# LessUp/n-body

Measured on AMD Instinct MI355X. Metric: pair_interactions_per_s, higher is better.
Workload: dtype f32; 1 GPU; plummer_N1048576_direct_n2_velocity_verlet; bodies=1048576, seed=42, deterministic=True, deterministic_mode=1

## Files before the change

n-body_amd/csrc/api.hip:

```cpp

#include <cstdarg>
#include <cstdlib>
#include <cstring>

#include "common.h"
#include "onesweep.h"

namespace nbh {

static thread_local char g_err[512] = "";

void set_error(const char* fmt, ...) {
  va_list ap;
  va_start(ap, fmt);
  vsnprintf(g_err, sizeof(g_err), fmt, ap);
  va_end(ap);
}

int fail(nbody_hip_status code, const char* file, int line, const char* fmt, ...) {
  char msg[384];
  va_list ap;
  va_start(ap, fmt);
  vsnprintf(msg, sizeof(msg), fmt, ap);
  va_end(ap);
  const char* base = strrchr(file, '/');
  snprintf(g_err, sizeof(g_err), "%s at %s:%d", msg, base ? base + 1 : file, line);
  return (int)code;
}

int Workspace::reserve(size_t want) {
  if (want <= bytes) return NBODY_HIP_OK;
  size_t cap = bytes + bytes / 2;
  if (cap < want) cap = want;
  cap = (cap + 255) & ~(size_t)255;
  want = (want + 255) & ~(size_t)255;
  if (ptr) {
    NBH_HIP(hipDeviceSynchronize());
    NBH_HIP(hipFree(ptr));
    ptr = nullptr;
    bytes = 0;
    generation++;
  }
  void* p = nullptr;
  hipError_t e = hipMalloc(&p, cap);
  if (e != hipSuccess && cap > want) {
    (void)hipGetLastError();
    cap = want;
    e = hipMalloc(&p, cap);
  }
  if (e != hipSuccess) {
    (void)hipGetLastError();
    return ::nbh::fail(e == hipErrorOutOfMemory ? NBODY_HIP_ERR_RESOURCE : NBODY_HIP_ERR_DEVICE, __FILE__, __LINE__,
                       "hipMalloc(%zu bytes of workspace): %s", cap, hipGetErrorString(e));
  }
  ptr = p;
  bytes = cap;
  generation++;
  return NBODY_HIP_OK;
}

void Workspace::release() {
  if (ptr) (void)hipFree(ptr);
  ptr = nullptr;
  bytes = 0;
  generation++;
}

}

using namespace nbh;

extern "C" int nbody_hip_abi_version(void) { return NBODY_HIP_ABI_VERSION; }

extern "C" int nbody_hip_sort_info(int* driver_compiled, int* self_test, int* own_self_test, int* rocprim_version) {
  if (driver_compiled) *driver_compiled = NBH_ONESWEEP_AVAILABLE;
  if (self_test) *self_test = nbh::driver_sort_verdict.state.load(std::memory_order_acquire);
  if (own_self_test) *own_self_test = nbh::own_sort_verdict.state.load(std::memory_order_acquire);
  if (rocprim_version) *rocprim_version = (int)ROCPRIM_VERSION;
  return NBODY_HIP_OK;
}

extern "C" const char* nbody_hip_last_error(void) { return g_err; }

extern "C" int nbody_hip_device_count(void) {
  int n = 0;
  if (hipGetDeviceCount(&n) != hipSuccess) {
    (void)hipGetLastError();
    return 0;
  }
  return n;
}

extern "C" int nbody_hip_ctx_create(nbody_hip_ctx** out, int device, void* stream) {
  if (!out) return NBH_FAIL(NBODY_HIP_ERR_STATE, "null output pointer");
  *out = nullptr;
  const int ndev = nbody_hip_device_count();
  if (ndev <= 0)
    return NBH_FAIL(NBODY_HIP_ERR_DEVICE, "no HIP device available (this library has no CPU fallback)");
  if (device < 0 || device >= ndev)
    return NBH_FAIL(NBODY_HIP_ERR_VALIDATION, "device %d out of range [0,%d)", device, ndev);
  NBH_HIP(hipSetDevice(device));
  nbody_hip_ctx* c = new nbody_hip_ctx();
  c->device = device;
  c->stream = static_cast<hipStream_t>(stream);
  hipError_t e = hipHostMalloc(reinterpret_cast<void**>(&c->host_scalar), 4 * sizeof(double), hipHostMallocDefault);
  if (e == hipSuccess) e = hipEventCreate(&c->ev0);
  if (e == hipSuccess) e = hipEventCreate(&c->ev1);
  if (e != hipSuccess) {
    nbody_hip_ctx_destroy(c);
    return NBH_FAIL(NBODY_HIP_ERR_DEVICE, "context resources: %s", hipGetErrorString(e));
  }
  *out = c;
  return NBODY_HIP_OK;
}

extern "C" int nbody_hip_ctx_destroy(nbody_hip_ctx* ctx) {
  if (!ctx) return NBODY_HIP_OK;
  NBH_DESTROY_BEGIN
  (void)hipSetDevice(ctx->device);
  (void)hipStreamSynchronize(ctx->stream);
  ctx->posm.release();
  ctx->partial.release();
  ctx->reduce.release();
  if (ctx->host_scalar) (void)hipHostFree(ctx->host_scalar);
  if (ctx->ev0) (void)hipEventDestroy(ctx->ev0);
  if (ctx->ev1) (void)hipEventDestroy(ctx->ev1);
  if (ctx->capture_stream) (void)hipStreamDestroy(ctx->capture_stream);
  delete ctx;
  NBH_DESTROY_END
}

extern "C" int nbody_hip_ctx_set_stream(nbody_hip_ctx* ctx, void* stream) {
  if (!ctx) return NBH_FAIL(NBODY_HIP_ERR_STATE, "null context");
  ctx->stream = static_cast<hipStream_t>(stream);
  return NBODY_HIP_OK;
}

extern "C" int nbody_hip_ctx_synchronize(nbody_hip_ctx* ctx) {
  if (!ctx) return NBH_FAIL(NBODY_HIP_ERR_STATE, "null context");
  NBH_NOT_CAPTURABLE(ctx, "nbody_hip_ctx_synchronize");
  NBH_HIP(hipSetDevice(ctx->device));
  NBH_HIP(hipStreamSynchronize(ctx->stream));
  return NBODY_HIP_OK;
}


struct nbody_hip_graph {
  nbody_hip_ctx* ctx = nullptr;
  hipGraph_t graph = nullptr;
  hipGraphExec_t exec = nullptr;
  unsigned long long generation = 0;
};

extern "C" int nbody_hip_capture_begin(nbody_hip_ctx* ctx) {
  if (!ctx) return NBH_FAIL(NBODY_HIP_ERR_STATE, "null context");
  if (ctx->capturing) return NBH_FAIL(NBODY_HIP_ERR_STATE, "capture already in progress");
  NBH_HIP(hipSetDevice(ctx->device));
  if (!ctx->capture_stream) NBH_HIP(hipStreamCreateWithFlags(&ctx->capture_stream, hipStreamNonBlocking));
  NBH_HIP(hipStreamSynchronize(ctx->stream));
  NBH_HIP(hipStreamBeginCapture(ctx->capture_stream, hipStreamCaptureModeThreadLocal));
  ctx->user_stream = ctx->stream;
  ctx->stream = ctx->capture_stream;
  ctx->capturing = true;
  ctx->capture_failed = false;
  return NBODY_HIP_OK;
}

extern "C" int nbody_hip_capture_end(nbody_hip_ctx* ctx, nbody_hip_graph** out) {
  if (!ctx || !out) return NBH_FAIL(NBODY_HIP_ERR_STATE, "null argument");
  *out = nullptr;
  if (!ctx->capturing) return NBH_FAIL(NBODY_HIP_ERR_STATE, "no capture in progress");
  hipGraph_t graph = nullptr;
  const hipError_t e = hipStreamEndCapture(ctx->capture_stream, &graph);
  ctx->stream = ctx->user_stream;
  ctx->capturing = false;
  if (e != hipSuccess || !graph || ctx->capture_failed) {
    (void)hipGetLastError();
    if (graph) (void)hipGraphDestroy(graph);
    return NBH_FAIL(NBODY_HIP_ERR_DEVICE, "hipStreamEndCapture: %s (a call inside the capture was not capturable)",
                    hipGetErrorString(e));
  }
  nbody_hip_graph* g = new nbody_hip_graph();
  g->ctx = ctx;
  g->graph = graph;
  g->generation = ctx->generation();
  const hipError_t ei = hipGraphInstantiate(&g->exec, graph, nullptr, nullptr, 0);
  if (ei != hipSuccess) {
    (void)hipGraphDestroy(graph);
    delete g;
    return NBH_FAIL(NBODY_HIP_ERR_DEVICE, "hipGraphInstantiate: %s", hipGetErrorString(ei));
  }
  *out = g;
  return NBODY_HIP_OK;
}

extern "C" int nbody_hip_graph_launch(nbody_hip_graph* g, int times) {
  if (!g || !g->exec) return NBH_FAIL(NBODY_HIP_ERR_STATE, "null graph");
  if (g->ctx->capturing) return NBH_FAIL(NBODY_HIP_ERR_STATE, "graph launch inside a capture");
  if (g->generation != g->ctx->generation())
    return NBH_FAIL(NBODY_HIP_ERR_STATE, "step graph is stale: device buffers of its context were re-allocated "
                    "after it was recorded (record it again)");
  NBH_HIP(hipSetDevice(g->ctx->device));
  g->ctx->graph_replays += (unsigned long long)(times > 0 ? times : 0);
  for (int i = 0; i < times; i++) NBH_HIP(hipGraphLaunch(g->exec, g->ctx->stream));
  return NBODY_HIP_OK;
}

extern "C" int nbody_hip_graph_destroy(nbody_hip_graph* g) {
  if (!g) return NBODY_HIP_OK;
  NBH_DESTROY_BEGIN
  (void)hipSetDevice(g->ctx->device);
  (void)hipStreamSynchronize(g->ctx->stream);
  if (g->exec) (void)hipGraphExecDestroy(g->exec);
  if (g->graph) (void)hipGraphDestroy(g->graph);
  delete g;
  NBH_DESTROY_END
}


static inline float** field(nbody_particle_data* d, int k) { return &d->pos_x + k; }
static inline float* const* cfield(const nbody_particle_data* d, int k) { return &d->pos_x + k; }

extern "C" int nbody_hip_particles_alloc(nbody_particle_data* d, size_t count) {
  if (!d) return NBH_FAIL(NBODY_HIP_ERR_STATE, "null particle data");
  if (count == 0) return NBH_FAIL(NBODY_HIP_ERR_VALIDATION, "Particle count must be greater than 0");
  if (count > 100000000u)
    return NBH_FAIL(NBODY_HIP_ERR_VALIDATION, "Particle count exceeds maximum supported (100M)");
  if (nbody_hip_device_count() <= 0)
    return NBH_FAIL(NBODY_HIP_ERR_DEVICE, "no HIP device available (this library has no CPU fallback)");
  const size_t stride = ((count * sizeof(float)) + 255) & ~(size_t)255;
  char* base = nullptr;
  NBH_HIP(hipMalloc(reinterpret_cast<void**>(&base), stride * 13));
  hipError_t e = hipMemset(base, 0, stride * 13);
  if (e != hipSuccess) {
    (void)hipFree(base);
    return NBH_FAIL(NBODY_HIP_ERR_DEVICE, "hipMemset: %s", hipGetErrorString(e));
  }
  for (int k = 0; k < 13; k++) *field(d, k) = reinterpret_cast<float*>(base + stride * k);
  d->count = count;
  return NBODY_HIP_OK;
}

extern "C" int nbody_hip_particles_free(nbody_particle_data* d) {
  if (!d) return NBODY_HIP_OK;
  if (d->pos_x) {
    NBH_HIP(hipDeviceSynchronize());
    NBH_HIP(hipFree(d->pos_x));
  }
  for (int k = 0; k < 13; k++) *field(d, k) = nullptr;
  d->count = 0;
  return NBODY_HIP_OK;
}

static const int kCopied[10] = {0, 1, 2, 3, 4, 5, 6, 7, 8, 12};

extern "C" int nbody_hip_particles_upload(nbody_particle_data* d, const nbody_particle_data* h) {
  if (!d || !h) return NBH_FAIL(NBODY_HIP_ERR_STATE, "null particle data");
  if (h->count > d->count)
    return NBH_FAIL(NBODY_HIP_ERR_VALIDATION, "host count %zu exceeds device capacity %zu", h->count, d->count);
  const size_t bytes = h->count * sizeof(float);
  for (int k : kCopied) {
    if (!*cfield(h, k) || !*cfield(d, k)) return NBH_FAIL(NBODY_HIP_ERR_STATE, "null array in particle data");
    NBH_HIP(hipMemcpy(*field(d, k), *cfield(h, k), bytes, hipMemcpyHostToDevice));
  }
  return NBODY_HIP_OK;
}

extern "C" int nbody_hip_particles_download(nbody_particle_data* h, const nbody_particle_data* d) {
  if (!d || !h) return NBH_FAIL(NBODY_HIP_ERR_STATE, "null particle data");
  if (d->count > h->count)
    return NBH_FAIL(NBODY_HIP_ERR_VALIDATION, "device count %zu exceeds host capacity %zu", d->count, h->count);
  const size_t bytes = d->count * sizeof(float);
  for (int k : kCopied) {
    if (!*cfield(h, k) || !*cfield(d, k)) return NBH_FAIL(NBODY_HIP_ERR_STATE, "null array in particle data");
    NBH_HIP(hipMemcpy(*field(h, k), *cfield(d, k), bytes, hipMemcpyDeviceToHost));
  }
  return NBODY_HIP_OK;
}


extern "C" int nbody_hip_pack_posm(nbody_hip_ctx* ctx, const float* x, const float* y,
                                   const float* z, const float* mass, size_t count,
                                   nbody_float4* out) {
  if (!ctx) return NBH_FAIL(NBODY_HIP_ERR_STATE, "null context");
  if (count == 0) return NBODY_HIP_OK;
  if (!x || !y || !z || !mass || !out) return NBH_FAIL(NBODY_HIP_ERR_STATE, "null argument");
  if (count > 0x3fffffffu) return NBH_FAIL(NBODY_HIP_ERR_VALIDATION, "body count exceeds 2^30");
  NBH_HIP(hipSetDevice(ctx->device));
  return pack_posm(ctx, x, y, z, mass, count, reinterpret_cast<float4*>(out));
}

namespace nbh {
__global__ __launch_bounds__(kBlock) void unpack3_kernel(const float4* __restrict__ in, int n,
                                                         float* __restrict__ x,
                                                         float* __restrict__ y,
                                                         float* __restrict__ z) {
  const int i = blockIdx.x * kBlock + threadIdx.x;
  if (i < n) {
    const float4 v = in[i];
    x[i] = v.x; y[i] = v.y; z[i] = v.z;
  }
}
}

extern "C" int nbody_hip_unpack3(nbody_hip_ctx* ctx, const nbody_float4* in, size_t count, float* x,
                                 float* y, float* z) {
  if (!ctx) return NBH_FAIL(NBODY_HIP_ERR_STATE, "null context");
  if (count == 0) return NBODY_HIP_OK;
  if (!x || !y || !z || !in) return NBH_FAIL(NBODY_HIP_ERR_STATE, "null argument");
  if (count > 0x3fffffffu) return NBH_FAIL(NBODY_HIP_ERR_VALIDATION, "body count exceeds 2^30");
  NBH_HIP(hipSetDevice(ctx->device));
  hipLaunchKernelGGL(unpack3_kernel, dim3((unsigned)((count + kBlock - 1) / kBlock)), dim3(kBlock),
                     0, ctx->stream, reinterpret_cast<const float4*>(in), (int)count, x, y, z);
  NBH_LAUNCH_CHECK();
  return NBODY_HIP_OK;
}

extern "C" int nbody_hip_direct_forces(nbody_hip_ctx* ctx, const nbody_particle_data* d, float G,
                                       float eps2, int block_size) {
  if (!ctx) return NBH_FAIL(NBODY_HIP_ERR_STATE, "null context");
  if (!d) return NBH_FAIL(NBODY_HIP_ERR_STATE, "null particle data");
  if (block_size <= 0 || block_size > 1024)
    return NBH_FAIL(NBODY_HIP_ERR_VALIDATION, "CUDA block size must be between 1 and 1024");
  const size_t n = d->count;
  if (n == 0) return NBODY_HIP_OK;
  if (!d->pos_x || !d->pos_y || !d->pos_z || !d->mass || !d->acc_x || !d->acc_y || !d->acc_z)
    return NBH_FAIL(NBODY_HIP_ERR_STATE, "particle data has null arrays");
  if (n > 0x3fffffffu) return NBH_FAIL(NBODY_HIP_ERR_VALIDATION, "body count exceeds 2^30");
  NBH_HIP(hipSetDevice(ctx->device));
  if (int rc = ctx->posm.reserve(n * sizeof(float4))) return rc;
  float4* posm = static_cast<float4*>(ctx->posm.ptr);
  if (int rc = pack_posm(ctx, d->pos_x, d->pos_y, d->pos_z, d->mass, n, posm)) return rc;
  return direct_packed(ctx, posm, n, posm, n, G, eps2, nullptr, 0, d->acc_x, d->acc_y, d->acc_z,
                       nullptr, nullptr, nullptr, nullptr, nullptr, nullptr, 0.f);
}

extern "C" int nbody_hip_direct_forces_packed(nbody_hip_ctx* ctx, const nbody_float4* targets,
                                              size_t n_targets, const nbody_float4* sources,
                                              size_t n_sources, nbody_float4* acc_out, float G,
                                              float eps2, int accumulate) {
  if (!ctx) return NBH_FAIL(NBODY_HIP_ERR_STATE, "null context");
  if (n_targets == 0) return NBODY_HIP_OK;
  if (!targets || !acc_out || (n_sources > 0 && !sources))
    return NBH_FAIL(NBODY_HIP_ERR_STATE, "null argument");
  NBH_HIP(hipSetDevice(ctx->device));
  return direct_packed(ctx, reinterpret_cast<const float4*>(targets), n_targets,
                       reinterpret_cast<const float4*>(sources), n_sources, G, eps2,
                       reinterpret_cast<float4*>(acc_out), accumulate, nullptr, nullptr, nullptr,
                       nullptr, nullptr, nullptr, nullptr, nullptr, nullptr, 0.f);
}

extern "C" int nbody_hip_direct_forces_pair_packed(nbody_hip_ctx* ctx, const nbody_float4* a, size_t n_a,
                                                   const nbody_float4* b, size_t n_b, nbody_float4* acc_a,
                                                   int accumulate_a, nbody_float4* acc_b, int accumulate_b,
                                                   float G, float eps2) {
  if (!ctx) return NBH_FAIL(NBODY_HIP_ERR_STATE, "null context");
  if (n_a == 0 || n_b == 0) return NBH_FAIL(NBODY_HIP_ERR_VALIDATION, "both body sets must be non-empty");
  if (!a || !b || !acc_a || !acc_b) return NBH_FAIL(NBODY_HIP_ERR_STATE, "null argument");
  if (n_a > 0x3fffffffu || n_b > 0x3fffffffu) return NBH_FAIL(NBODY_HIP_ERR_VALIDATION, "body count exceeds 2^30");
  if (!(eps2 >= 1e-12f))
    return NBH_FAIL(NBODY_HIP_ERR_VALIDATION, "pair evaluation needs eps2 >= 1e-12 (use the one-sided entry point)");
  NBH_HIP(hipSetDevice(ctx->device));
  return direct_symmetric_pair(ctx, reinterpret_cast<const float4*>(a), n_a, reinterpret_cast<const float4*>(b),
                               n_b, G, eps2, reinterpret_cast<float4*>(acc_a), accumulate_a,
                               reinterpret_cast<float4*>(acc_b), accumulate_b);
}

extern "C" int nbody_hip_time_direct_packed(nbody_hip_ctx* ctx, const nbody_float4* targets,
                                            size_t n_targets, const nbody_float4* sources,
                                            size_t n_sources, nbody_float4* acc_out, float G,
                                            float eps2, int iters, float* ms_per_launch) {
  if (!ctx) return NBH_FAIL(NBODY_HIP_ERR_STATE, "null context");
  if (!ms_per_launch || iters <= 0) return NBH_FAIL(NBODY_HIP_ERR_VALIDATION, "bad timing arguments");
  NBH_HIP(hipSetDevice(ctx->device));
  if (int rc = nbody_hip_direct_forces_packed(ctx, targets, n_targets, sources, n_sources, acc_out, G, eps2, 0))
    return rc;
  NBH_HIP(hipEventRecord(ctx->ev0, ctx->stream));
  for (int i = 0; i < iters; i++)
    if (int rc = nbody_hip_direct_forces_packed(ctx, targets, n_targets, sources, n_sources, acc_out, G, eps2, 0))
      return rc;
  NBH_HIP(hipEventRecord(ctx->ev1, ctx->stream));
  NBH_HIP(hipEventSynchronize(ctx->ev1));
  float ms = 0.f;
  NBH_HIP(hipEventElapsedTime(&ms, ctx->ev0, ctx->ev1));
  *ms_per_launch = ms / (float)iters;
  return NBODY_HIP_OK;
}

extern "C" int nbody_hip_direct_deterministic(nbody_hip_ctx* ctx, int mode) {
  if (!ctx) return NBH_FAIL(NBODY_HIP_ERR_STATE, "null context");
  if (mode < 0 || mode > 2) return NBH_FAIL(NBODY_HIP_ERR_VALIDATION, "mode must be 0 (atomics), 1 (slots when they fit) or 2 (slots required)");
  ctx->deterministic = mode;
  if (mode == 0 && ctx->partial.bytes > ((size_t)64 << 20) && !ctx->capturing) {
    NBH_HIP(hipSetDevice(ctx->device));
    NBH_HIP(hipDeviceSynchronize());
    ctx->partial.release();
  }
  return NBODY_HIP_OK;
}

extern "C" int nbody_hip_direct_slot_budget(nbody_hip_ctx* ctx, unsigned long long bytes) {
  if (!ctx) return NBH_FAIL(NBODY_HIP_ERR_STATE, "null context");
  ctx->det_budget = bytes ? (size_t)bytes : ((size_t)24 << 30);
  return NBODY_HIP_OK;
}

extern "C" int nbody_hip_direct_info(nbody_hip_ctx* ctx, size_t count, float eps2, nbody_hip_direct_info_t* out) {
  if (!out) return NBH_FAIL(NBODY_HIP_ERR_STATE, "null argument");
  const nbody_hip_ctx defaults{};
  const nbody_hip_ctx* c = ctx ? ctx : &defaults;
  memset(out, 0, sizeof(*out));
  out->deterministic_mode = c->deterministic;
  out->last_kernel = c->last_direct_kernel;
  out->workspace_bytes_held = c->partial.bytes;
  if (count == 0) return NBODY_HIP_OK;
  if (count > 0x3fffffffu) return NBH_FAIL(NBODY_HIP_ERR_VALIDATION, "body count exceeds 2^30");
  const bool dev = ctx && nbody_hip_device_count() > 0 && hipSetDevice(ctx->device) == hipSuccess;
  DirectPlan p = direct_plan(c, count, dev);
  if (!(eps2 >= 1e-12f)) p.symmetric = false;
  if (!p.symmetric) {
    out->kernel = 0;
    return NBODY_HIP_OK;
  }
  out->kernel = p.det ? 2 : 1;
  out->bodies_per_lane_equal = p.eq.R;
  out->bodies_per_lane_general = p.gen.R;
  out->reaction_slots = p.det ? p.eq.D : 0;
  out->iside_slots = p.det ? p.eq.splits : 1;
  out->workspace_bytes_needed = p.bytes;
  out->slot_bytes_wanted = p.det_bytes_wanted;
  return NBODY_HIP_OK;
}

extern "C" int nbody_hip_direct_tuning(nbody_hip_ctx* ctx, int variant, int targets_per_lane,
                                       int source_splits) {
  if (!ctx) return NBH_FAIL(NBODY_HIP_ERR_STATE, "null context");
  if (variant < -1 || variant > 3) return NBH_FAIL(NBODY_HIP_ERR_VALIDATION, "variant must be -1 (auto), 0, 1, 2 or 3");
  if (targets_per_lane != 0 && targets_per_lane != 1 && targets_per_lane != 2 && targets_per_lane != 4 &&
      targets_per_lane != 6 && targets_per_lane != 8 && targets_per_lane != 12 && targets_per_lane != 16)
    return NBH_FAIL(NBODY_HIP_ERR_VALIDATION, "targets_per_lane must be 0 (auto), 1, 2, 4 (6, 8, 16: symmetric kernel only)");
  if (source_splits < 0 || source_splits > 4096)
    return NBH_FAIL(NBODY_HIP_ERR_VALIDATION, "source_splits must be in [0, 4096]");
  ctx->tune_variant = variant;
  ctx->tune_tpl = targets_per_lane;
  ctx->tune_splits = source_splits;
  return NBODY_HIP_OK;
}
```

n-body_amd/csrc/direct_sym.hip:

```cpp

#include <type_traits>

#include "common.h"

namespace nbh {

typedef float f2 __attribute__((ext_vector_type(2)));

__device__ __forceinline__ float wave_rot1(float v) {
  return __int_as_float(__builtin_amdgcn_mov_dpp(__float_as_int(v), 0x134 , 0xF, 0xF, false));
}

constexpr int kSymBlocksPerCU = 16;
constexpr int kSymMinChunks = 4;
constexpr float kFar = 1.0e18f;

template <int R, bool RECT, bool EQM, bool DET = false>
__global__ __launch_bounds__(kBlock) void direct_sym_kernel(const float4* __restrict__ posm, int n,
                                                            const float4* __restrict__ posj, int nj,
                                                            int NB, int NBJ, int chunks_per_split,
                                                            double* __restrict__ acc64,
                                                            void* __restrict__ accj,
                                                            size_t plane_i, size_t plane_j,
                                                            const unsigned int* __restrict__ mass_range,
                                                            float eps2) {
  const bool uniform = mass_range[0] == mass_range[1] && mass_range[2] == mass_range[3] &&
                       mass_range[0] == mass_range[2] && ordered_to_float(mass_range[0]) > 0.f;
  if (uniform != EQM) return;
  const float m0 = EQM ? ordered_to_float(mass_range[0]) : 1.0f;
  constexpr int S = kBlock * R;
  __shared__ float slab[2][4][3][64];
  const int tid = threadIdx.x, lane = tid & 63, w = tid >> 6;
  const int A = blockIdx.x;
  const int D = RECT ? NBJ - 1 : NB / 2;
  constexpr int CPB = kBlock * R / 64;
  const int q0 = blockIdx.y * chunks_per_split;
  const int q1 = min((D + 1) * CPB, q0 + chunks_per_split);
  if (q0 >= q1) {
    if constexpr (DET) {
#pragma unroll
      for (int r = 0; r < R; r++)
#pragma unroll
        for (int c = 0; c < 3; c++)
          acc64[((size_t)blockIdx.y * 3 + c) * plane_i + (size_t)(A * S + r * kBlock + tid)] = 0.0;
    }
    return;
  }

  f2 xi[R / 2], yi[R / 2], zi[R / 2], mi[R / 2];
#pragma unroll
  for (int r = 0; r < R / 2; r++) {
    float4 p0 = make_float4(kFar, kFar, kFar, 0.f), p1 = p0;
    const int i0 = A * S + (2 * r) * kBlock + tid, i1 = i0 + kBlock;
    if (i0 < n) p0 = posm[i0];
    if (i1 < n) p1 = posm[i1];
    xi[r] = f2{p0.x, p1.x}; yi[r] = f2{p0.y, p1.y}; zi[r] = f2{p0.z, p1.z}; mi[r] = f2{p0.w, p1.w};
  }
  constexpr bool LACC = R >= 8;
  constexpr int RR = LACC ? 1 : R;
  __shared__ double lacc[LACC ? 3 * R * kBlock : 1];
  double sx[RR], sy[RR], sz[RR];
  if constexpr (LACC) {
#pragma unroll
    for (int k = 0; k < 3 * R; k++) lacc[k * kBlock + tid] = 0.0;
  } else {
#pragma unroll
    for (int r = 0; r < R; r++) sx[r] = sy[r] = sz[r] = 0.0;
  }
  f2 ax[R / 2], ay[R / 2], az[R / 2];
#pragma unroll
  for (int r = 0; r < R / 2; r++) ax[r] = ay[r] = az[r] = f2{0.f, 0.f};
  const f2 e2 = {eps2, eps2};

  auto partner_valid = [&](int d) { return RECT || !((NB % 2 == 0) && d == D && d > 0 && A >= D); };
  const int nchunks = q1 - q0;

  auto load_chunk = [&](int q) -> float4 {
    const int d = (q0 + q) / CPB, c = (q0 + q) % CPB;
    const int B = RECT ? d : (A + d) % NB;
    const int j = B * S + c * 64 + lane;
    float4 p = make_float4(kFar, kFar, kFar, 0.f);
    if (RECT) { if (j < nj) p = posj[j]; }
    else if (j < n && partner_valid(d)) p = posm[j];
    return p;
  };
  auto flush_chunk = [&](int q) {
    const int pd = (q0 + q) / CPB, pc = (q0 + q) % CPB;
    if constexpr (DET) {
      if (RECT || pd > 0) {
        const size_t plane = RECT ? plane_j : plane_i;
        float* slot = static_cast<float*>(accj) + (size_t)(RECT ? A : pd - 1) * 3 * plane;
        const unsigned int j = (unsigned int)((RECT ? pd : (A + pd) % NB) * S + pc * 64 + lane), pl = (unsigned int)plane;
        const int sb = q & 1;
        const bool keep = partner_valid(pd);
#pragma unroll
        for (int c = 0; c < 3; c++) {
          const float v = (slab[sb][0][c][lane] + slab[sb][1][c][lane]) + (slab[sb][2][c][lane] + slab[sb][3][c][lane]);
          slot[c * pl + j] = keep ? v : 0.f;
        }
      }
    } else if ((RECT || pd > 0) && partner_valid(pd)) {
      const int j = (RECT ? pd : (A + pd) % NB) * S + pc * 64 + lane;
      const int sb = q & 1;
      double* dst = RECT ? static_cast<double*>(accj) : acc64;
      const size_t plane = RECT ? plane_j : plane_i;
#pragma unroll
      for (int c = 0; c < 3; c++) {
        const float v = (slab[sb][0][c][lane] + slab[sb][1][c][lane]) + (slab[sb][2][c][lane] + slab[sb][3][c][lane]);
        unsafeAtomicAdd(&dst[c * plane + (size_t)j], (double)v * (double)m0);
      }
    }
  };

  float4 jnext = load_chunk(0);
  for (int q = 0; q < nchunks; q++) {
    const float4 jcur = jnext;
    if (q + 1 < nchunks) jnext = load_chunk(q + 1);
    const int d = (q0 + q) / CPB;
    const bool react = RECT || d > 0;
    if (q > 0) {
      __syncthreads();
      if (w == (q & 3)) flush_chunk(q - 1);
    }
    float jx = jcur.x, jy = jcur.y, jz = jcur.z, jm = jcur.w;
    float hjx = 0.f, hjy = 0.f, hjz = 0.f;
    auto steps = [&](auto react_tag) {
      constexpr bool REACT = decltype(react_tag)::value;
      constexpr int kStepUnroll = R >= 16 ? 1 : 2;
#pragma unroll kStepUnroll
      for (int k = 0; k < 64; k++) {
        const f2 sxj = {jx, jx}, syj = {jy, jy}, szj = {jz, jz}, smj = {jm, jm};
        f2 dx[R / 2], dy[R / 2], dz[R / 2], g[R / 2];
#pragma unroll
        for (int r = 0; r < R / 2; r++) {
          dx[r] = sxj - xi[r]; dy[r] = syj - yi[r]; dz[r] = szj - zi[r];
          g[r] = __builtin_elementwise_fma(dx[r], dx[r], __builtin_elementwise_fma(dy[r], dy[r], __builtin_elementwise_fma(dz[r], dz[r], e2)));
        }
#pragma unroll
        for (int r = 0; r < R / 2; r++) {
          g[r].x = __builtin_amdgcn_rsqf(g[r].x);
          g[r].y = __builtin_amdgcn_rsqf(g[r].y);
        }
#pragma unroll
        for (int r = 0; r < R / 2; r++) g[r] = (g[r] * g[r]) * g[r];
        f2 hx = {hjx, 0.f}, hy = {hjy, 0.f}, hz = {hjz, 0.f};
#pragma unroll
        for (int r = 0; r < R / 2; r++) {
          const f2 fj = EQM ? g[r] : g[r] * smj;
          ax[r] = __builtin_elementwise_fma(fj, dx[r], ax[r]);
          ay[r] = __builtin_elementwise_fma(fj, dy[r], ay[r]);
          az[r] = __builtin_elementwise_fma(fj, dz[r], az[r]);
          if (REACT) {
            const f2 fi = EQM ? g[r] : g[r] * mi[r];
            hx = __builtin_elementwise_fma(-fi, dx[r], hx);
            hy = __builtin_elementwise_fma(-fi, dy[r], hy);
            hz = __builtin_elementwise_fma(-fi, dz[r], hz);
          }
        }
        if (REACT) {
          hjx = wave_rot1(hx.x + hx.y); hjy = wave_rot1(hy.x + hy.y); hjz = wave_rot1(hz.x + hz.y);
        }
        jx = wave_rot1(jx); jy = wave_rot1(jy); jz = wave_rot1(jz); jm = wave_rot1(jm);
      }
    };
    if constexpr (R >= 12 && !EQM) {
      (void)react;
      steps(std::true_type{});
    } else {
      if (react) steps(std::true_type{}); else steps(std::false_type{});
    }
    slab[q & 1][w][0][lane] = hjx; slab[q & 1][w][1][lane] = hjy; slab[q & 1][w][2][lane] = hjz;
    if ((q & 3) == 3 || q == nchunks - 1) {
#pragma unroll
      for (int r = 0; r < R / 2; r++) {
        if constexpr (LACC) {
          lacc[(0 * R + 2 * r) * kBlock + tid] += (double)ax[r].x; lacc[(0 * R + 2 * r + 1) * kBlock + tid] += (double)ax[r].y;
          lacc[(1 * R + 2 * r) * kBlock + tid] += (double)ay[r].x; lacc[(1 * R + 2 * r + 1) * kBlock + tid] += (double)ay[r].y;
          lacc[(2 * R + 2 * r) * kBlock + tid] += (double)az[r].x; lacc[(2 * R + 2 * r + 1) * kBlock + tid] += (double)az[r].y;
        } else {
          sx[2 * r] += (double)ax[r].x; sx[2 * r + 1] += (double)ax[r].y;
          sy[2 * r] += (double)ay[r].x; sy[2 * r + 1] += (double)ay[r].y;
          sz[2 * r] += (double)az[r].x; sz[2 * r + 1] += (double)az[r].y;
        }
        ax[r] = ay[r] = az[r] = f2{0.f, 0.f};
      }
    }
  }
  __syncthreads();
  if (w == (nchunks & 3)) flush_chunk(nchunks - 1);
#pragma unroll
  for (int r = 0; r < R; r++) {
    const int i = A * S + r * kBlock + tid;
    const double fx = LACC ? lacc[(0 * R + r) * kBlock + tid] : sx[LACC ? 0 : r];
    const double fy = LACC ? lacc[(1 * R + r) * kBlock + tid] : sy[LACC ? 0 : r];
    const double fz = LACC ? lacc[(2 * R + r) * kBlock + tid] : sz[LACC ? 0 : r];
    if constexpr (DET) {
      double* slot = acc64 + (size_t)blockIdx.y * 3 * plane_i;
      const unsigned int iu = (unsigned int)i, pl = (unsigned int)plane_i;
      slot[iu] = fx;
      slot[pl + iu] = fy;
      slot[2u * pl + iu] = fz;
    } else {
      unsafeAtomicAdd(&acc64[(size_t)i], fx * (double)m0);
      unsafeAtomicAdd(&acc64[plane_i + (size_t)i], fy * (double)m0);
      unsafeAtomicAdd(&acc64[2 * plane_i + (size_t)i], fz * (double)m0);
    }
  }
}

__global__ void mass_range_init_kernel(unsigned int* enc) {
  if (threadIdx.x < 4) enc[threadIdx.x] = (threadIdx.x & 1) ? 0u : 0xffffffffu;
}

__global__ __launch_bounds__(kBlock) void mass_range_kernel(const float4* __restrict__ posm, int n,
                                                            unsigned int* __restrict__ enc) {
  __shared__ float red[4][2];
  float lo = INFINITY, hi = -INFINITY;
  for (int i = blockIdx.x * kBlock + threadIdx.x; i < n; i += gridDim.x * kBlock) {
    const float m = posm[i].w;
    lo = fminf(lo, m); hi = fmaxf(hi, m);
  }
#pragma unroll
  for (int off = 32; off > 0; off >>= 1) {
    lo = fminf(lo, __shfl_down(lo, off, 64));
    hi = fmaxf(hi, __shfl_down(hi, off, 64));
  }
  const int w = threadIdx.x >> 6;
  if ((threadIdx.x & 63) == 0) { red[w][0] = lo; red[w][1] = hi; }
  __syncthreads();
  if (threadIdx.x == 0) {
    for (int k = 1; k < 4; k++) { lo = fminf(lo, red[k][0]); hi = fmaxf(hi, red[k][1]); }
    atomicMin(&enc[0], float_to_ordered(fminf(lo, red[0][0])));
    atomicMax(&enc[1], float_to_ordered(fmaxf(hi, red[0][1])));
  }
}

struct SlotLayout {
  const double* isl;
  const float* rsl;
  size_t plane;
  int n_i, n_r;
};

__global__ __launch_bounds__(kBlock) void direct_sym_finalize_kernel(
    SlotLayout eq, SlotLayout gen, int apply_m0, const unsigned int* __restrict__ mass_range, int n, float G,
    float4* __restrict__ acc4, int accumulate, float* __restrict__ ax, float* __restrict__ ay, float* __restrict__ az,
    float* __restrict__ vx, float* __restrict__ vy, float* __restrict__ vz, const float* __restrict__ aox,
    const float* __restrict__ aoy, const float* __restrict__ aoz, float half_dt) {
  const int i = blockIdx.x * kBlock + threadIdx.x;
  if (i >= n) return;
  SlotLayout L = eq;
  double m0 = 1.0;
  if (mass_range) {
    const bool uniform = mass_range[0] == mass_range[1] && mass_range[2] == mass_range[3] &&
                         mass_range[0] == mass_range[2] && ordered_to_float(mass_range[0]) > 0.f;
    if (!uniform) L = gen;
    else if (apply_m0) m0 = (double)ordered_to_float(mass_range[0]);
  }
  double sx = 0.0, sy = 0.0, sz = 0.0;
  for (int k = 0; k < L.n_r; k++) {
    const float* p = L.rsl + (size_t)k * 3 * L.plane;
    sx += (double)p[i]; sy += (double)p[L.plane + i]; sz += (double)p[2 * L.plane + i];
  }
  for (int k = 0; k < L.n_i; k++) {
    const double* p = L.isl + (size_t)k * 3 * L.plane;
    sx += p[i]; sy += p[L.plane + i]; sz += p[2 * L.plane + i];
  }
  const double gm = (double)G * m0;
  const float fx = (float)(gm * sx), fy = (float)(gm * sy), fz = (float)(gm * sz);
  if (acc4) {
    float4 o = make_float4(fx, fy, fz, 0.f);
    if (accumulate) { const float4 c = acc4[i]; o.x += c.x; o.y += c.y; o.z += c.z; }
    acc4[i] = o;
  } else {
    ax[i] = fx; ay[i] = fy; az[i] = fz;
    if (vx) {
      vx[i] = kick1(vx[i], aox[i], fx, half_dt);
      vy[i] = kick1(vy[i], aoy[i], fy, half_dt);
      vz[i] = kick1(vz[i], aoz[i], fz, half_dt);
    }
  }
}

static void launch_mass_range(nbody_hip_ctx* ctx, const float4* pi, int ni, const float4* pj, int nj,
                              unsigned int* enc) {
  hipLaunchKernelGGL(mass_range_init_kernel, dim3(1), dim3(64), 0, ctx->stream, enc);
  const int bi = (ni + kBlock - 1) / kBlock, bj = (nj + kBlock - 1) / kBlock;
  hipLaunchKernelGGL(mass_range_kernel, dim3(bi < 256 ? bi : 256), dim3(kBlock), 0, ctx->stream, pi, ni, enc);
  hipLaunchKernelGGL(mass_range_kernel, dim3(bj < 256 ? bj : 256), dim3(kBlock), 0, ctx->stream, pj, nj, enc + 2);
}

template <int R, bool RECT, bool DET>
static void launch_sym(nbody_hip_ctx* ctx, dim3 grid, const float4* pi, int ni, const float4* pj, int nj,
                       int NB, int NBJ, int per, double* acci, void* accj, const unsigned int* enc,
                       float eps2) {
  const size_t S = (size_t)kBlock * R;
  hipLaunchKernelGGL((direct_sym_kernel<R, RECT, true, DET>), grid, dim3(kBlock), 0, ctx->stream, pi, ni, pj, nj,
                     NB, NBJ, per, acci, accj, (size_t)NB * S, (size_t)NBJ * S, enc, eps2);
  hipLaunchKernelGGL((direct_sym_kernel<R, RECT, false, DET>), grid, dim3(kBlock), 0, ctx->stream, pi, ni, pj, nj,
                     NB, NBJ, per, acci, accj, (size_t)NB * S, (size_t)NBJ * S, enc, eps2);
}

bool symmetric_pays(const nbody_hip_ctx* ctx, size_t n) {
  if (ctx->tune_variant == 3) return true;
  return ctx->tune_variant < 0 && n >= 12288;
}

static int sym_R(const nbody_hip_ctx* ctx, size_t n, bool two_sets) {
  if (ctx->tune_tpl == 2 || ctx->tune_tpl == 4 || ctx->tune_tpl == 6 || ctx->tune_tpl == 8 ||
      ctx->tune_tpl == 16 || (ctx->tune_tpl == 12 && !two_sets))
    return ctx->tune_tpl;
  if (two_sets) return n >= 49152 ? 16 : (n >= 16384 ? 8 : 4);
  return n >= 200000 ? 16 : (n >= 100000 ? 12 : (n >= 28000 ? 8 : 6));
}

static size_t align256(size_t b) { return (b + 255) & ~(size_t)255; }

SymShape sym_shape(const nbody_hip_ctx* ctx, size_t n, int R) {
  SymShape c;
  c.R = R;
  const int S = kBlock * R;
  c.NB = (int)((n + S - 1) / S);
  c.D = c.NB / 2;
  const int total = (c.D + 1) * (S / 64);
  int splits = ctx->tune_splits > 0 ? ctx->tune_splits : (kNumCU * kSymBlocksPerCU + c.NB - 1) / c.NB;
  if (splits < 1) splits = 1;
  int per = (total + splits - 1) / splits;
  if (per < kSymMinChunks) per = kSymMinChunks;
  if (per > S / 64) per = (per + S / 64 - 1) / (S / 64) * (S / 64);
  c.per = per;
  c.splits = (total + per - 1) / per;
  c.plane = (size_t)c.NB * S;
  return c;
}
size_t SymShape::reaction_bytes() const { return align256((size_t)D * 3 * plane * sizeof(float)); }
size_t SymShape::det_bytes() const { return reaction_bytes() + (size_t)splits * 3 * plane * sizeof(double); }
size_t SymShape::atomic_bytes() const { return 3 * plane * sizeof(double); }

static bool det_budget_allows(const nbody_hip_ctx* ctx, size_t bytes, size_t* free_now) {
  if (free_now) *free_now = 0;
  if (bytes > ctx->det_budget) return false;
  if (bytes <= ctx->partial.bytes) return true;
  size_t free_b = 0, total_b = 0;
  if (hipMemGetInfo(&free_b, &total_b) != hipSuccess) {
    (void)hipGetLastError();
    return true;
  }
  if (free_now) *free_now = free_b;
  return bytes <= (free_b + ctx->partial.bytes) / 4;
}

DirectPlan direct_plan(const nbody_hip_ctx* ctx, size_t n, bool query_device) {
  DirectPlan p;
  p.symmetric = symmetric_pays(ctx, n);
  p.eq = sym_shape(ctx, n, sym_R(ctx, n, false));
  p.gen = p.eq;
  p.det = false;
  p.bytes = 0;
  if (!p.symmetric) return p;
  if (ctx->deterministic) {
    SymShape gen = (kDetGenR != 16 && p.eq.R == 16 && ctx->tune_tpl == 0) ? sym_shape(ctx, n, kDetGenR) : p.eq;
    size_t need = p.eq.det_bytes() > gen.det_bytes() ? p.eq.det_bytes() : gen.det_bytes();
    bool ok = query_device ? det_budget_allows(ctx, need, nullptr) : need <= ctx->det_budget;
    if (!ok && gen.R != p.eq.R) {
      gen = p.eq;
      need = p.eq.det_bytes();
      ok = query_device ? det_budget_allows(ctx, need, nullptr) : need <= ctx->det_budget;
    }
    if (ok) {
      p.det = true;
      p.gen = gen;
      p.bytes = need;
    }
    p.det_bytes_wanted = need;
  }
  if (!p.det) p.bytes = p.eq.atomic_bytes();
  return p;
}

namespace {
template <int R, bool EQM, bool DET>
void launch_all_pairs(nbody_hip_ctx* ctx, const SymShape& c, const float4* posm, int n, double* acci, void* accj,
                      const unsigned int* enc, float eps2) {
  hipLaunchKernelGGL((direct_sym_kernel<R, false, EQM, DET>), dim3(c.NB, c.splits), dim3(kBlock), 0, ctx->stream, posm, n,
                     posm, n, c.NB, c.NB, c.per, acci, accj, c.plane, c.plane, enc, eps2);
}
template <bool EQM, bool DET>
void launch_all_pairs_R(nbody_hip_ctx* ctx, const SymShape& c, const float4* posm, int n, double* acci, void* accj,
                        const unsigned int* enc, float eps2) {
  switch (c.R) {
    case 2: launch_all_pairs<2, EQM, DET>(ctx, c, posm, n, acci, accj, enc, eps2); break;
    case 6: launch_all_pairs<6, EQM, DET>(ctx, c, posm, n, acci, accj, enc, eps2); break;
    case 8: launch_all_pairs<8, EQM, DET>(ctx, c, posm, n, acci, accj, enc, eps2); break;
    case 12: launch_all_pairs<12, EQM, DET>(ctx, c, posm, n, acci, accj, enc, eps2); break;
    case 16: launch_all_pairs<16, EQM, DET>(ctx, c, posm, n, acci, accj, enc, eps2); break;
    default: launch_all_pairs<4, EQM, DET>(ctx, c, posm, n, acci, accj, enc, eps2); break;
  }
}
}

int direct_symmetric(nbody_hip_ctx* ctx, const float4* posm, size_t n, float G, float eps2,
                     float4* acc4, int accumulate, float* ax, float* ay, float* az, float* vx,
                     float* vy, float* vz, const float* aox, const float* aoy, const float* aoz,
                     float half_dt) {
  DirectPlan plan = direct_plan(ctx, n, true);
  if (ctx->deterministic == 2 && !plan.det)
    return NBH_FAIL(NBODY_HIP_ERR_RESOURCE, "deterministic Direct sums were required but their slot planes (%zu bytes "
                    "for %zu bodies) exceed the budget (%zu bytes and a quarter of the free device memory)",
                    plan.det_bytes_wanted, n, ctx->det_budget);
  if (ctx->partial.bytes > ((size_t)64 << 20) && ctx->partial.bytes / 4 > plan.bytes && !ctx->capturing) {
    NBH_HIP(hipDeviceSynchronize());
    ctx->partial.release();
  }
  int rc = ctx->partial.reserve(plan.bytes);
  if (rc != NBODY_HIP_OK && plan.det && ctx->deterministic != 2) {
    (void)hipGetLastError();
    plan.det = false;
    plan.gen = plan.eq;
    plan.bytes = plan.eq.atomic_bytes();
    rc = ctx->partial.reserve(plan.bytes);
  }
  if (rc != NBODY_HIP_OK) return rc;
  const SymShape &eq = plan.eq, &gen = plan.gen;
  const bool det = plan.det;
  char* base = static_cast<char*>(ctx->partial.ptr);
  if (!det) NBH_HIP(hipMemsetAsync(base, 0, plan.bytes, ctx->stream));
  if (int rc2 = ctx->reduce.reserve(64)) return rc2;
  unsigned int* enc = static_cast<unsigned int*>(ctx->reduce.ptr);
  const int ni = (int)n;
  launch_mass_range(ctx, posm, ni, posm, ni, enc);
  SlotLayout Leq, Lgen;
  if (det) {
    Leq = SlotLayout{reinterpret_cast<const double*>(base + eq.reaction_bytes()), reinterpret_cast<const float*>(base),
                     eq.plane, eq.splits, eq.D};
    Lgen = SlotLayout{reinterpret_cast<const double*>(base + gen.reaction_bytes()), reinterpret_cast<const float*>(base),
                      gen.plane, gen.splits, gen.D};
    launch_all_pairs_R<true, true>(ctx, eq, posm, ni, const_cast<double*>(Leq.isl), base, enc, eps2);
    launch_all_pairs_R<false, true>(ctx, gen, posm, ni, const_cast<double*>(Lgen.isl), base, enc, eps2);
  } else {
    Leq = Lgen = SlotLayout{reinterpret_cast<const double*>(base), nullptr, eq.plane, 1, 0};
    launch_all_pairs_R<true, false>(ctx, eq, posm, ni, reinterpret_cast<double*>(base), base, enc, eps2);
    launch_all_pairs_R<false, false>(ctx, gen, posm, ni, reinterpret_cast<double*>(base), base, enc, eps2);
  }
  NBH_LAUNCH_CHECK();
  ctx->last_direct_kernel = det ? 2 : 1;
  const int fblocks = (int)((n + kBlock - 1) / kBlock);
  hipLaunchKernelGGL(direct_sym_finalize_kernel, dim3(fblocks), dim3(kBlock), 0, ctx->stream, Leq, Lgen, det ? 1 : 0, enc,
                     ni, G, acc4, accumulate, ax, ay, az, vx, vy, vz, aox, aoy, aoz, half_dt);
  NBH_LAUNCH_CHECK();
  return NBODY_HIP_OK;
}

int direct_symmetric_pair(nbody_hip_ctx* ctx, const float4* pi, size_t ni, const float4* pj, size_t nj,
                          float G, float eps2, float4* acc_i, int accumulate_i, float4* acc_j,
                          int accumulate_j) {
  int R = 0, NBI = 0, NBJ = 0, per = 0, splits = 0;
  size_t plane_i = 0, plane_j = 0, det_i = 0, det_j = 0;
  auto shape = [&](bool det_form) {
    const size_t nmin = ni < nj ? ni : nj;
    R = sym_R(ctx, nmin, true);
    if (det_form && ctx->tune_tpl == 0 && R > 8) R = 8;
    const int S = kBlock * R;
    NBI = (int)((ni + S - 1) / S);
    NBJ = (int)((nj + S - 1) / S);
    const int total = NBJ * (S / 64);
    const int per_cu = det_form ? kSymBlocksPerCU / 2 : kSymBlocksPerCU;
    splits = ctx->tune_splits > 0 ? ctx->tune_splits : (kNumCU * per_cu + NBI - 1) / NBI;
    if (splits < 1) splits = 1;
    per = (total + splits - 1) / splits;
    if (per < kSymMinChunks) per = kSymMinChunks;
    if (per > S / 64) per = (per + S / 64 - 1) / (S / 64) * (S / 64);
    splits = (total + per - 1) / per;
    plane_i = (size_t)NBI * S;
    plane_j = (size_t)NBJ * S;
    det_i = align256((size_t)splits * 3 * plane_i * sizeof(double));
    det_j = (size_t)NBI * 3 * plane_j * sizeof(float);
  };
  shape(ctx->deterministic != 0);
  bool det = ctx->deterministic != 0 && det_budget_allows(ctx, det_i + det_j, nullptr);
  if (ctx->deterministic == 2 && !det)
    return NBH_FAIL(NBODY_HIP_ERR_RESOURCE, "deterministic Direct sums were required but their slot planes (%zu bytes) "
                    "exceed the budget", det_i + det_j);
  if (!det) shape(false);
  size_t bi = align256(plane_i * 3 * sizeof(double)), bj = plane_j * 3 * sizeof(double);
  int rc = ctx->partial.reserve(det ? det_i + det_j : bi + bj);
  if (rc != NBODY_HIP_OK && det && ctx->deterministic != 2) {
    (void)hipGetLastError();
    det = false;
    shape(false);
    bi = align256(plane_i * 3 * sizeof(double));
    bj = plane_j * 3 * sizeof(double);
    rc = ctx->partial.reserve(bi + bj);
  }
  if (rc != NBODY_HIP_OK) return rc;
  char* base = static_cast<char*>(ctx->partial.ptr);
  double* acci = reinterpret_cast<double*>(base);
  void* accj = base + (det ? det_i : bi);
  if (!det) NBH_HIP(hipMemsetAsync(base, 0, bi + bj, ctx->stream));
  if (int rc2 = ctx->reduce.reserve(64)) return rc2;
  unsigned int* enc = static_cast<unsigned int*>(ctx->reduce.ptr);
  launch_mass_range(ctx, pi, (int)ni, pj, (int)nj, enc);
  const dim3 grid(NBI, splits);
#define NBH_PAIR_LAUNCH(RR)                                                                                          \
  if (det) launch_sym<RR, true, true>(ctx, grid, pi, (int)ni, pj, (int)nj, NBI, NBJ, per, acci, accj, enc, eps2);    \
  else launch_sym<RR, true, false>(ctx, grid, pi, (int)ni, pj, (int)nj, NBI, NBJ, per, acci, accj, enc, eps2)
  switch (R) {
    case 2: NBH_PAIR_LAUNCH(2); break;
    case 6: NBH_PAIR_LAUNCH(6); break;
    case 8: NBH_PAIR_LAUNCH(8); break;
    case 16: NBH_PAIR_LAUNCH(16); break;
    default: NBH_PAIR_LAUNCH(4); break;
  }
#undef NBH_PAIR_LAUNCH
  NBH_LAUNCH_CHECK();
  ctx->last_direct_kernel = det ? 2 : 1;
  SlotLayout Li, Lj;
  if (det) {
    Li = SlotLayout{acci, nullptr, plane_i, splits, 0};
    Lj = SlotLayout{nullptr, static_cast<const float*>(accj), plane_j, 0, NBI};
  } else {
    Li = SlotLayout{acci, nullptr, plane_i, 1, 0};
    Lj = SlotLayout{static_cast<const double*>(accj), nullptr, plane_j, 1, 0};
  }
  hipLaunchKernelGGL(direct_sym_finalize_kernel, dim3((unsigned)((ni + kBlock - 1) / kBlock)), dim3(kBlock), 0,
                     ctx->stream, Li, Li, det ? 1 : 0, det ? enc : nullptr, (int)ni, G, acc_i, accumulate_i, nullptr, nullptr,
                     nullptr, nullptr, nullptr, nullptr, nullptr, nullptr, nullptr, 0.f);
  hipLaunchKernelGGL(direct_sym_finalize_kernel, dim3((unsigned)((nj + kBlock - 1) / kBlock)), dim3(kBlock), 0,
                     ctx->stream, Lj, Lj, det ? 1 : 0, det ? enc : nullptr, (int)nj, G, acc_j, accumulate_j, nullptr, nullptr,
                     nullptr, nullptr, nullptr, nullptr, nullptr, nullptr, nullptr, 0.f);
  NBH_LAUNCH_CHECK();
  return NBODY_HIP_OK;
}

}
```

Measured before the change: 7004 billion pair-interactions/s.

## Split R=16 symmetric accumulators between LDS and registers for two workgroups per CU

For the R=16 symmetric direct kernel, only 12 of the 16 targets' double accumulators stay in LDS and the other 4 move to registers. This shrinks LDS per workgroup so two workgroups can share a CU, and launch_bounds is raised to match. For equal masses, the inner step loop is split into two half-phases to lower live VGPR pressure. The old all-LDS path stays available as tuning variant 4. The risk is register spills from the added double accumulators under the tighter launch bound.

```diff
diff --git a/n-body_amd/csrc/api.hip b/n-body_amd/csrc/api.hip
--- a/n-body_amd/csrc/api.hip
+++ b/n-body_amd/csrc/api.hip
@@ -435,7 +435,7 @@
 extern "C" int nbody_hip_direct_tuning(nbody_hip_ctx* ctx, int variant, int targets_per_lane,
                                        int source_splits) {
   if (!ctx) return NBH_FAIL(NBODY_HIP_ERR_STATE, "null context");
-  if (variant < -1 || variant > 3) return NBH_FAIL(NBODY_HIP_ERR_VALIDATION, "variant must be -1 (auto), 0, 1, 2 or 3");
+  if (variant < -1 || variant > 4) return NBH_FAIL(NBODY_HIP_ERR_VALIDATION, "variant must be -1 (auto), 0, 1, 2, 3 or 4");
   if (targets_per_lane != 0 && targets_per_lane != 1 && targets_per_lane != 2 && targets_per_lane != 4 &&
       targets_per_lane != 6 && targets_per_lane != 8 && targets_per_lane != 12 && targets_per_lane != 16)
     return NBH_FAIL(NBODY_HIP_ERR_VALIDATION, "targets_per_lane must be 0 (auto), 1, 2, 4 (6, 8, 16: symmetric kernel only)");
diff --git a/n-body_amd/csrc/direct_sym.hip b/n-body_amd/csrc/direct_sym.hip
--- a/n-body_amd/csrc/direct_sym.hip
+++ b/n-body_amd/csrc/direct_sym.hip
@@ -15,8 +15,9 @@
 constexpr int kSymMinChunks = 4;
 constexpr float kFar = 1.0e18f;
 
-template <int R, bool RECT, bool EQM, bool DET = false>
-__global__ __launch_bounds__(kBlock) void direct_sym_kernel(const float4* __restrict__ posm, int n,
+constexpr int sym_RL(int R) { return R >= 16 ? 12 : (R >= 8 ? R : 0); }
+template <int R, bool RECT, bool EQM, bool DET = false, int RL = sym_RL(R)>
+__global__ __launch_bounds__(kBlock, (R >= 16 && RL < R) ? 2 : 1) void direct_sym_kernel(const float4* __restrict__ posm, int n,
                                                             const float4* __restrict__ posj, int nj,
                                                             int NB, int NBJ, int chunks_per_split,
                                                             double* __restrict__ acc64,
@@ -56,17 +57,16 @@
     if (i1 < n) p1 = posm[i1];
     xi[r] = f2{p0.x, p1.x}; yi[r] = f2{p0.y, p1.y}; zi[r] = f2{p0.z, p1.z}; mi[r] = f2{p0.w, p1.w};
   }
-  constexpr bool LACC = R >= 8;
-  constexpr int RR = LACC ? 1 : R;
-  __shared__ double lacc[LACC ? 3 * R * kBlock : 1];
-  double sx[RR], sy[RR], sz[RR];
-  if constexpr (LACC) {
-#pragma unroll
-    for (int k = 0; k < 3 * R; k++) lacc[k * kBlock + tid] = 0.0;
-  } else {
-#pragma unroll
-    for (int r = 0; r < R; r++) sx[r] = sy[r] = sz[r] = 0.0;
-  }
+  static_assert(RL >= 0 && RL <= R && RL % 2 == 0, "whole packed pairs on either side");
+  static_assert(R < 12 || RL == R || 3 * RL * kBlock * sizeof(double) + sizeof(slab) <= 80 * 1024,
+                "two workgroups per CU need <= 80 KiB of LDS each");
+  constexpr int RG = R - RL;
+  __shared__ double lacc[RL > 0 ? 3 * RL * kBlock : 1];
+  double sx[RG > 0 ? RG : 1], sy[RG > 0 ? RG : 1], sz[RG > 0 ? RG : 1];
+#pragma unroll
+  for (int k = 0; k < 3 * RL; k++) lacc[k * kBlock + tid] = 0.0;
+#pragma unroll
+  for (int r = 0; r < RG; r++) sx[r] = sy[r] = sz[r] = 0.0;
   f2 ax[R / 2], ay[R / 2], az[R / 2];
 #pragma unroll
   for (int r = 0; r < R / 2; r++) ax[r] = ay[r] = az[r] = f2{0.f, 0.f};
@@ -127,35 +127,46 @@
     auto steps = [&](auto react_tag) {
       constexpr bool REACT = decltype(react_tag)::value;
       constexpr int kStepUnroll = R >= 16 ? 1 : 2;
+      constexpr int PH = (R >= 16 && RL < R && EQM) ? R / 4 : R / 2;
 #pragma unroll kStepUnroll
       for (int k = 0; k < 64; k++) {
         const f2 sxj = {jx, jx}, syj = {jy, jy}, szj = {jz, jz}, smj = {jm, jm};
-        f2 dx[R / 2], dy[R / 2], dz[R / 2], g[R / 2];
-#pragma unroll
-        for (int r = 0; r < R / 2; r++) {
-          dx[r] = sxj - xi[r]; dy[r] = syj - yi[r]; dz[r] = szj - zi[r];
-          g[r] = __builtin_elementwise_fma(dx[r], dx[r], __builtin_elementwise_fma(dy[r], dy[r], __builtin_elementwise_fma(dz[r], dz[r], e2)));
-        }
-#pragma unroll
-        for (int r = 0; r < R / 2; r++) {
-          g[r].x = __builtin_amdgcn_rsqf(g[r].x);
-          g[r].y = __builtin_amdgcn_rsqf(g[r].y);
-        }
-#pragma unroll
-        for (int r = 0; r < R / 2; r++) g[r] = (g[r] * g[r]) * g[r];
+        f2 dx[PH], dy[PH], dz[PH], g[PH];
+        auto phase_g = [&](int b) {
+#pragma unroll
+          for (int r = 0; r < PH; r++) {
+            dx[r] = sxj - xi[b + r]; dy[r] = syj - yi[b + r]; dz[r] = szj - zi[b + r];
+            g[r] = __builtin_elementwise_fma(dx[r], dx[r], __builtin_elementwise_fma(dy[r], dy[r], __builtin_elementwise_fma(dz[r], dz[r], e2)));
+          }
+#pragma unroll
+          for (int r = 0; r < PH; r++) {
+            g[r].x = __builtin_amdgcn_rsqf(g[r].x);
+            g[r].y = __builtin_amdgcn_rsqf(g[r].y);
+          }
+#pragma unroll
+          for (int r = 0; r < PH; r++) g[r] = (g[r] * g[r]) * g[r];
+        };
+        phase_g(0);
         f2 hx = {hjx, 0.f}, hy = {hjy, 0.f}, hz = {hjz, 0.f};
-#pragma unroll
-        for (int r = 0; r < R / 2; r++) {
-          const f2 fj = EQM ? g[r] : g[r] * smj;
-          ax[r] = __builtin_elementwise_fma(fj, dx[r], ax[r]);
-          ay[r] = __builtin_elementwise_fma(fj, dy[r], ay[r]);
-          az[r] = __builtin_elementwise_fma(fj, dz[r], az[r]);
-          if (REACT) {
-            const f2 fi = EQM ? g[r] : g[r] * mi[r];
-            hx = __builtin_elementwise_fma(-fi, dx[r], hx);
-            hy = __builtin_elementwise_fma(-fi, dy[r], hy);
-            hz = __builtin_elementwise_fma(-fi, dz[r], hz);
+        auto phase_sums = [&](int b) {
+#pragma unroll
+          for (int r = 0; r < PH; r++) {
+            const f2 fj = EQM ? g[r] : g[r] * smj;
+            ax[b + r] = __builtin_elementwise_fma(fj, dx[r], ax[b + r]);
+            ay[b + r] = __builtin_elementwise_fma(fj, dy[r], ay[b + r]);
+            az[b + r] = __builtin_elementwise_fma(fj, dz[r], az[b + r]);
+            if (REACT) {
+              const f2 fi = EQM ? g[r] : g[r] * mi[b + r];
+              hx = __builtin_elementwise_fma(-fi, dx[r], hx);
+              hy = __builtin_elementwise_fma(-fi, dy[r], hy);
+              hz = __builtin_elementwise_fma(-fi, dz[r], hz);
+            }
           }
+        };
+        phase_sums(0);
+        if constexpr (PH < R / 2) {
+          phase_g(PH);
+          phase_sums(PH);
         }
         if (REACT) {
           hjx = wave_rot1(hx.x + hx.y); hjy = wave_rot1(hy.x + hy.y); hjz = wave_rot1(hz.x + hz.y);
@@ -173,14 +184,14 @@
     if ((q & 3) == 3 || q == nchunks - 1) {
 #pragma unroll
       for (int r = 0; r < R / 2; r++) {
-        if constexpr (LACC) {
-          lacc[(0 * R + 2 * r) * kBlock + tid] += (double)ax[r].x; lacc[(0 * R + 2 * r + 1) * kBlock + tid] += (double)ax[r].y;
-          lacc[(1 * R + 2 * r) * kBlock + tid] += (double)ay[r].x; lacc[(1 * R + 2 * r + 1) * kBlock + tid] += (double)ay[r].y;
-          lacc[(2 * R + 2 * r) * kBlock + tid] += (double)az[r].x; lacc[(2 * R + 2 * r + 1) * kBlock + tid] += (double)az[r].y;
+        if (2 * r < RL) {
+          lacc[(0 * RL + 2 * r) * kBlock + tid] += (double)ax[r].x; lacc[(0 * RL + 2 * r + 1) * kBlock + tid] += (double)ax[r].y;
+          lacc[(1 * RL + 2 * r) * kBlock + tid] += (double)ay[r].x; lacc[(1 * RL + 2 * r + 1) * kBlock + tid] += (double)ay[r].y;
+          lacc[(2 * RL + 2 * r) * kBlock + tid] += (double)az[r].x; lacc[(2 * RL + 2 * r + 1) * kBlock + tid] += (double)az[r].y;
         } else {
-          sx[2 * r] += (double)ax[r].x; sx[2 * r + 1] += (double)ax[r].y;
-          sy[2 * r] += (double)ay[r].x; sy[2 * r + 1] += (double)ay[r].y;
-          sz[2 * r] += (double)az[r].x; sz[2 * r + 1] += (double)az[r].y;
+          sx[2 * r - RL] += (double)ax[r].x; sx[2 * r + 1 - RL] += (double)ax[r].y;
+          sy[2 * r - RL] += (double)ay[r].x; sy[2 * r + 1 - RL] += (double)ay[r].y;
+          sz[2 * r - RL] += (double)az[r].x; sz[2 * r + 1 - RL] += (double)az[r].y;
         }
         ax[r] = ay[r] = az[r] = f2{0.f, 0.f};
       }
@@ -191,9 +202,9 @@
 #pragma unroll
   for (int r = 0; r < R; r++) {
     const int i = A * S + r * kBlock + tid;
-    const double fx = LACC ? lacc[(0 * R + r) * kBlock + tid] : sx[LACC ? 0 : r];
-    const double fy = LACC ? lacc[(1 * R + r) * kBlock + tid] : sy[LACC ? 0 : r];
-    const double fz = LACC ? lacc[(2 * R + r) * kBlock + tid] : sz[LACC ? 0 : r];
+    const double fx = r < RL ? lacc[(0 * RL + r) * kBlock + tid] : sx[r < RL ? 0 : r - RL];
+    const double fy = r < RL ? lacc[(1 * RL + r) * kBlock + tid] : sy[r < RL ? 0 : r - RL];
+    const double fz = r < RL ? lacc[(2 * RL + r) * kBlock + tid] : sz[r < RL ? 0 : r - RL];
     if constexpr (DET) {
       double* slot = acc64 + (size_t)blockIdx.y * 3 * plane_i;
       const unsigned int iu = (unsigned int)i, pl = (unsigned int)plane_i;
@@ -290,19 +301,32 @@
   hipLaunchKernelGGL(mass_range_kernel, dim3(bj < 256 ? bj : 256), dim3(kBlock), 0, ctx->stream, pj, nj, enc + 2);
 }
 
+template <int R, bool RECT, bool DET, int RL>
+static void launch_sym_rl(nbody_hip_ctx* ctx, dim3 grid, const float4* pi, int ni, const float4* pj, int nj,
+                          int NB, int NBJ, int per, double* acci, void* accj, const unsigned int* enc,
+                          float eps2) {
+  const size_t S = (size_t)kBlock * R;
+  hipLaunchKernelGGL((direct_sym_kernel<R, RECT, true, DET, RL>), grid, dim3(kBlock), 0, ctx->stream, pi, ni, pj, nj,
+                     NB, NBJ, per, acci, accj, (size_t)NB * S, (size_t)NBJ * S, enc, eps2);
+  hipLaunchKernelGGL((direct_sym_kernel<R, RECT, false, DET, RL>), grid, dim3(kBlock), 0, ctx->stream, pi, ni, pj, nj,
+                     NB, NBJ, per, acci, accj, (size_t)NB * S, (size_t)NBJ * S, enc, eps2);
+}
+
+constexpr int kPairRL16 = 12;
+
 template <int R, bool RECT, bool DET>
 static void launch_sym(nbody_hip_ctx* ctx, dim3 grid, const float4* pi, int ni, const float4* pj, int nj,
                        int NB, int NBJ, int per, double* acci, void* accj, const unsigned int* enc,
                        float eps2) {
-  const size_t S = (size_t)kBlock * R;
-  hipLaunchKernelGGL((direct_sym_kernel<R, RECT, true, DET>), grid, dim3(kBlock), 0, ctx->stream, pi, ni, pj, nj,
-                     NB, NBJ, per, acci, accj, (size_t)NB * S, (size_t)NBJ * S, enc, eps2);
-  hipLaunchKernelGGL((direct_sym_kernel<R, RECT, false, DET>), grid, dim3(kBlock), 0, ctx->stream, pi, ni, pj, nj,
-                     NB, NBJ, per, acci, accj, (size_t)NB * S, (size_t)NBJ * S, enc, eps2);
+  if constexpr (R == 16 && !DET) {
+    if (ctx->tune_variant != 4)
+      return launch_sym_rl<R, RECT, DET, kPairRL16>(ctx, grid, pi, ni, pj, nj, NB, NBJ, per, acci, accj, enc, eps2);
+  }
+  launch_sym_rl<R, RECT, DET, (R >= 8 ? R : 0)>(ctx, grid, pi, ni, pj, nj, NB, NBJ, per, acci, accj, enc, eps2);
 }
 
 bool symmetric_pays(const nbody_hip_ctx* ctx, size_t n) {
-  if (ctx->tune_variant == 3) return true;
+  if (ctx->tune_variant == 3 || ctx->tune_variant == 4) return true;
   return ctx->tune_variant < 0 && n >= 12288;
 }
 
@@ -379,11 +403,14 @@
 }
 
 namespace {
-template <int R, bool EQM, bool DET>
+template <bool EQM, bool DET>
+constexpr int kSymRL16 = 12;
+
+template <int R, bool EQM, bool DET, int RL = sym_RL(R)>
 void launch_all_pairs(nbody_hip_ctx* ctx, const SymShape& c, const float4* posm, int n, double* acci, void* accj,
                       const unsigned int* enc, float eps2) {
-  hipLaunchKernelGGL((direct_sym_kernel<R, false, EQM, DET>), dim3(c.NB, c.splits), dim3(kBlock), 0, ctx->stream, posm, n,
-                     posm, n, c.NB, c.NB, c.per, acci, accj, c.plane, c.plane, enc, eps2);
+  hipLaunchKernelGGL((direct_sym_kernel<R, false, EQM, DET, RL>), dim3(c.NB, c.splits), dim3(kBlock), 0, ctx->stream,
+                     posm, n, posm, n, c.NB, c.NB, c.per, acci, accj, c.plane, c.plane, enc, eps2);
 }
 template <bool EQM, bool DET>
 void launch_all_pairs_R(nbody_hip_ctx* ctx, const SymShape& c, const float4* posm, int n, double* acci, void* accj,
@@ -393,7 +420,10 @@
     case 6: launch_all_pairs<6, EQM, DET>(ctx, c, posm, n, acci, accj, enc, eps2); break;
     case 8: launch_all_pairs<8, EQM, DET>(ctx, c, posm, n, acci, accj, enc, eps2); break;
     case 12: launch_all_pairs<12, EQM, DET>(ctx, c, posm, n, acci, accj, enc, eps2); break;
-    case 16: launch_all_pairs<16, EQM, DET>(ctx, c, posm, n, acci, accj, enc, eps2); break;
+    case 16:
+      if (ctx->tune_variant == 4) launch_all_pairs<16, EQM, DET, 16>(ctx, c, posm, n, acci, accj, enc, eps2);
+      else launch_all_pairs<16, EQM, DET, kSymRL16<EQM, DET>>(ctx, c, posm, n, acci, accj, enc, eps2);
+      break;
     default: launch_all_pairs<4, EQM, DET>(ctx, c, posm, n, acci, accj, enc, eps2); break;
   }
 }
```

Result: faster. 7277 billion pair-interactions/s, median of 6 (+3.9%).
